# DiamondLightSource/fast-feedback-service

Hardware: AMD Instinct MI355X
Metric: detector frames/s (Eiger-16M 4362x4148 uint16) (higher is better)
Workload: dtype u16; 1 GPU; eiger16m: 4148x4362 uint16, 7x7 dispersion window, 32 frames/step/GPU resident in HBM, spots+centroids returned to host; streams=4, parallelism=single GPU, spot_gather=none (single GPU)

## Files before the change

fast-feedback-service_amd/csrc/ffs_context.hip:

```cpp
#include <sys/mman.h>

#include "ffs_internal.hpp"
#include "kernels_mask.hpp"

static_assert(sizeof(ReflOut) == sizeof(ffs_reflection), "record layout");
static_assert(offsetof(ReflOut, sum_intensity) == offsetof(ffs_reflection, sum_intensity), "record layout");

thread_local std::string g_create_error;

static void ctx_destroy_internal(ffs_ctx* c);
namespace {
struct Registry {
    std::mutex mu;
    std::unordered_set<const void*> live[3];
    std::atomic<bool> exiting{false};
    bool exit_hook_installed = false;
};
Registry& registry() {
    static Registry* r = new Registry();
    return *r;
}
static void on_process_exit() {
    Registry& r = registry();
    std::vector<ffs_ctx*> ctxs;
// ... 131 lines not shown
    L.bpitch = (uint32_t)L.pitch_px;
    L.frame_stride = (uint64_t)L.pitch * height;
    L.plane_frame_stride = (uint64_t)L.mpitch * height;
    L.bytes_frame_stride = (uint64_t)L.bpitch * height;
    if (L.frame_stride >= (1ull << 32)) {
        g_create_error = "frame larger than 4 GiB";
        delete c;
        return FFS_ERR_INVALID;
    }
    const uint64_t npx = (uint64_t)width * height;
    c->cap = max_strong ? max_strong : (uint32_t)std::min<uint64_t>(npx, 1u << 18);
    c->cap = (uint32_t)std::min<uint64_t>(c->cap, npx);
    c->max_comp = std::min<uint32_t>(c->cap, 1u << 14);
    c->n_tiles = ((int)height + kTileRows - 1) / kTileRows;
    ffs_default_params(&c->params);
    if (hipSetDevice(device) != hipSuccess) {
        g_create_error = "hipSetDevice failed";
        delete c;
        return FFS_ERR_DEVICE;
    }
    hipError_t e = hipMalloc(&c->d_maskbits, L.plane_frame_stride + 256);
    if (e == hipSuccess) e = hipMalloc(&c->d_ginfo, (size_t)(L.H + kInfoExtraRows) * ((size_t)L.pitch_px * pixel_bytes / 4) + 256);
    if (e == hipSuccess) e = hipMalloc(&c->d_mmap, (size_t)L.H * L.pitch_px + 256);
    if (e != hipSuccess) {
        g_create_error = std::string("hipMalloc(mask): ") + hipGetErrorString(e);
        ctx_destroy_internal(c);
        return FFS_ERR_NOMEM;
    }
    c->chain_ok = chain_prepare_device();
    {
        int lo = 0, hi = 0;
        hipError_t es = hipDeviceGetStreamPriorityRange(&lo, &hi);
        if (es == hipSuccess) es = hipStreamCreateWithPriority(&c->dense_st, hipStreamNonBlocking, (lo + hi) / 2);
        if (es == hipSuccess) es = hipStreamCreateWithFlags(&c->up_st, hipStreamNonBlocking);
        for (auto& sp : c->sparse_st)
            if (es == hipSuccess) es = hipStreamCreateWithPriority(&sp, hipStreamNonBlocking, hi);
        if (es == hipSuccess)
            for (auto& e : c->chain_ev)
                if (es == hipSuccess) es = hipEventCreate(&e);
        if (es != hipSuccess) {
            g_create_error = std::string("creating the context's HIP streams: ") + hipGetErrorString(es);
            ctx_destroy_internal(c);
            return FFS_ERR_DEVICE;
        }
    }
    int rc = ffs_ctx_set_mask(c, nullptr);
// ... 80 lines not shown
    for (ffs_stream* s : streams)
        if (handle_take(kHandleStream, s)) stream_destroy_internal(s);
    for (ffs_stack3d* st : stacks)
        if (handle_take(kHandleStack, st)) {
            g_live_stacks.fetch_sub(1);
            stack3d_free(st);
        }
    ctx_destroy_internal(c);
}

static void ctx_destroy_internal(ffs_ctx* c) {
    (void)hipSetDevice(c->device);
    ahead_stop(c, true);
    for (auto* st : c->stack_pool) stack3d_free(st);
    c->stack_pool.clear();
    if (AssemblyPool* pool = c->assembly.exchange(nullptr)) {
        pool->owner.lock();
        pool->owner.unlock();
        delete pool;
    }
    if (c->d_maskbits) (void)hipFree(c->d_maskbits);
    if (c->d_ginfo) (void)hipFree(c->d_ginfo);
    if (c->d_mmap) (void)hipFree(c->d_mmap);
    if (c->dense_st) (void)hipStreamDestroy(c->dense_st);
    if (c->dense_st2) (void)hipStreamDestroy(c->dense_st2);
    if (c->d_handoff) (void)hipFree(c->d_handoff);
    if (c->up_st) (void)hipStreamDestroy(c->up_st);
    for (auto st : c->sparse_st) if (st) (void)hipStreamDestroy(st);
    for (auto e : c->chain_ev) if (e) (void)hipEventDestroy(e);
    for (auto& pb : c->pinned_pool) pinned_free(pb);
    delete c;
}

static int rebuild_mask_tables(ffs_ctx* c) {
    const Layout& L = c->L;
    const uint32_t gpitch = (uint32_t)L.pitch_px * (uint32_t)c->pixel_bytes / 4;
    HIP_TRY(c, hipMemset(c->d_ginfo, 0, (size_t)(L.H + kInfoExtraRows) * gpitch));
    const int groups = L.pitch_px / (c->pixel_bytes == 2 ? 8 : 4);
    (void)hipGetLastError();
    if (c->pixel_bytes == 2)
        hipLaunchKernelGGL(k_build_maps, dim3((groups + 255) / 256, L.H), dim3(256), 0, 0, c->d_maskbits, L.mpitch, L.W, L.H,
                           L.pitch_px, c->d_mmap, c->d_ginfo, gpitch);
    else
        hipLaunchKernelGGL(k_build_maps4, dim3((groups + 255) / 256, L.H), dim3(256), 0, 0, c->d_maskbits, L.mpitch, L.W, L.H,
                           L.pitch_px, c->d_mmap, c->d_ginfo, gpitch);
    HIP_TRY(c, hipGetLastError());
    HIP_TRY(c, hipDeviceSynchronize());
    return FFS_OK;
}

static int ffs_ctx_set_mask_impl(ffs_ctx* c, const uint8_t* host_mask) {
    if (!c) return FFS_ERR_INVALID;
    const Layout& L = c->L;
    std::vector<uint8_t> bits(L.plane_frame_stride, 0);
    const int full = L.W / 8;
    for (int y = 0; y < L.H; ++y) {
        uint8_t* row = bits.data() + (size_t)y * L.mpitch;
        if (host_mask) {
            const uint8_t* m = host_mask + (size_t)y * L.W;
            for (int g = 0; g < full; ++g) {
                uint64_t v;
                std::memcpy(&v, m + 8 * g, 8);
                const uint64_t nz = (((v & 0x7F7F7F7F7F7F7F7Full) + 0x7F7F7F7F7F7F7F7Full) | v) & 0x8080808080808080ull;
                row[g] = (uint8_t)(((nz >> 7) * 0x0102040810204080ull) >> 56);
            }
            for (int x = full * 8; x < L.W; ++x)
                if (m[x]) row[x >> 3] |= (uint8_t)(1u << (x & 7));
        } else {
// ... 60 lines not shown

extern "C" int ffs_ctx_device_layout(const ffs_ctx* c, size_t* pitch, size_t* fstride) {
    if (!c) return FFS_ERR_INVALID;
    if (pitch) *pitch = c->L.pitch;
    if (fstride) *fstride = c->L.frame_stride;
    return FFS_OK;
}

extern "C" int ffs_ctx_set_tuning(ffs_ctx* c, const char* key, long long value) {
    if (!c || !key) return FFS_ERR_INVALID;
    Tuning& t = c->tune;
    const std::string k = key;
    auto in = [&](long long lo, long long hi) { return value >= lo && value <= hi; };
    bool ok = true;
    if (k == "threshold_path") { if ((ok = in(0, 2))) t.threshold_path = (int)value; }
    else if (k == "window_kernel") { if ((ok = in(0, 1))) t.window_kernel = (int)value; }
    else if (k == "ext_first_pass") { if ((ok = value == 0 || value == 2)) t.ext_first_pass = (int)value; }
    else if (k == "sparse_stage") { if ((ok = in(1, 3))) t.sparse_stage = (int)value; }
    else if (k == "device_lists") { if ((ok = in(0, 2))) t.device_lists = (int)value; }
    else if (k == "strong_log") { if ((ok = in(0, 1))) t.strong_log = (int)value; }
    else if (k == "chain_runs") { if ((ok = in(0, 2))) t.chain_runs = (int)value; }
    else if (k == "dense_overlap") { if ((ok = in(0, 1))) t.dense_overlap = (int)value; }
    else if (k == "stream_prio") { if ((ok = in(0, 3))) t.stream_prio = (int)value; }
    else if (k == "wait_ahead") { if ((ok = in(0, 1))) t.wait_ahead = (int)value; }
    else if (k == "assembly_threads") { if ((ok = in(1, 31))) t.assembly_threads = (int)value; }
    else if (k == "sparse_bands") { if ((ok = in(0, 2))) t.sparse_bands = (int)value; }
    else if (k == "sparse_priority") {
        if ((ok = in(0, 2) && c->n_streams_made == 0)) {
            int lo = 0, hi = 0;
            HIP_TRY(c, hipSetDevice(c->device));
            HIP_TRY(c, hipDeviceGetStreamPriorityRange(&lo, &hi));
            const int prio = value == 0 ? hi : value == 1 ? lo : (lo + hi) / 2;
            for (auto& sp : c->sparse_st) {
                if (sp) (void)hipStreamDestroy(sp);
                sp = nullptr;
                HIP_TRY(c, hipStreamCreateWithPriority(&sp, hipStreamNonBlocking, prio));
            }
            t.sparse_priority = (int)value;
        }
    }
    else if (k == "sched") { if ((ok = (value == 0 || value == 3) && c->n_streams_made == 0)) t.sched = (int)value; }
    else if (k == "chain_first") { if ((ok = in(0, 64))) t.chain_first = (int)value; }
    else if (k == "bright_cap") { if ((ok = in(0, kBrightCap))) t.bright_cap = (int)value; }
    else if (k == "frames_per_group") { if ((ok = in(1, 1 << 30))) t.frames_per_group = (int)value; }
    else if (k == "target_waves") { if ((ok = in(1, 1 << 24))) t.target_waves = value; }
    else if (k == "stream_bands") { if ((ok = in(0, 4096))) t.stream_bands = (int)value; }
// ... 284 lines not shown
```

fast-feedback-service_amd/csrc/ffs_device.h:

```cpp
#pragma once
#include <hip/hip_runtime.h>
#include <stdint.h>

#ifdef FFS_EXPERIMENTS
#define FFS_DBG(args, bit) (((args).dbg & (bit)) != 0)
#define FFS_STOP_AFTER(A, phase) if ((A).stop_after == (phase)) return
#define FFS_PHASE_TS(A, idx) do { if ((A).phase_ts && threadIdx.x == 0) (A).phase_ts[(size_t)blockIdx.x * 8 + (idx)] = wall_clock64(); } while (0)
#else
#define FFS_PHASE_TS(A, idx) do {} while (0)
#define FFS_DBG(args, bit) false
#define FFS_STOP_AFTER(A, phase) do {} while (0)
#endif

namespace ffsamd {

struct Layout {
    int W, H;
    int pitch_px;
    uint32_t pitch;
    uint32_t mpitch;
    uint32_t bpitch;
    uint64_t frame_stride;
    uint64_t plane_frame_stride;
    uint64_t bytes_frame_stride;
};

constexpr int kSOwned = 62;
__host__ __device__ inline int band_first_row(int band, int band_rows, int band_rows2, int band_split) {
    return band < band_split ? band * band_rows : band_split * band_rows + (band - band_split) * band_rows2;
}
constexpr int kWinOwned = 62;
constexpr int kInfoExtraRows = 3;

constexpr int kWlogCap = 256;
constexpr int kTileRows = 8;
constexpr int kExactListCap = 2048;

struct ThresholdArgs {
    const void* image;
    uint64_t frame_stride;
    uint32_t pitch;
    const uint8_t* maskbits;
    uint8_t* bits;
    uint8_t* strong_bytes;
    uint32_t* tile_counts;
    int W, H, pitch_px;
    uint32_t mpitch, bpitch;
    uint64_t plane_frame_stride, bytes_frame_stride;
    int n_strips, band_rows, n_bands, n_tiles;
    int band_rows2, band_split;
    float kS;
    float kB;
    int min_count;
    double nsig_b, nsig_s, threshold;
    double nsig_b2, nsig_s2;
    long long max_valid;
    int int_pred;
    uint32_t ib2, is2;
    uint32_t thr_floor;
    int bright_to_plane;
    uint8_t* dplane;
    uint8_t* eplane;
    int eplane_clean;
    int ext_strips, ext_band_rows, ext_bands;
    int ext_flavour;
    int ext_variant;
    const uint8_t* ginfo;
    const uint8_t* mmap;
    uint32_t gpitch;
    int gpf;
    int n_frames;
    int group_frames;
    int s_strips, s_band_rows, s_bands;
    uint32_t* bright_n;
    uint2* bright_list;
    uint32_t bright_cap;
    uint32_t* overflow;
    uint32_t* occ;
    uint32_t occ_frame_words;
    uint32_t occ_spr;
    int dense_mask;
    uint2* wlog;
    uint32_t* wlog_n;
    uint4* wpix;
    uint32_t* handoff;
    uint32_t handoff_seq;
    int dbg_prio;
    int dbg;
    int kx, ky;
    int w_strips, w_band_rows, w_bands;
    float w_kS, w_kB;
};
// ... 148 lines not shown
```

fast-feedback-service_amd/csrc/ffs_internal.hpp:

```cpp
#pragma once
#include <algorithm>
#include <atomic>
#include <chrono>
#include <condition_variable>
#include <functional>
#include <cmath>
#include <cstdio>
#include <cstdlib>
#include <cstring>
#include <deque>
#include <map>
#include <mutex>
#include <new>
#include <string>
#include <thread>
#include <unordered_set>
#include <vector>

#include <hip/hip_runtime.h>
#include <hip/hip_ext.h>

#include "ffs_hip.h"
#include "ffs_device.h"

// ... 19 lines not shown
    int sched = 3;
    int chain_first = 2;
    int bright_cap = 1 << 20;
    int frames_per_group = 1 << 30;
    long long target_waves = 16384;
    int stream_bands = 0;
    int dense_mask = 0;
    int occupancy_bitmap = 1;
    int direct_records = 1;
    int decode_in_dense_stream = 1;
    int ccl_grid = 32;
    int ext_erode = 2;
    int ext_e_sparse = 0;
    int ext_fused = 0;
    int ext_rest_aside = 0;
    int band_taper = 0;
    int rows_ahead = 3;
    int device_lists = 2;
    int strong_log = 1;
    int chain_runs = 1;
    int sparse_bands = 1;
    int dense_overlap = 0;
    int stream_prio = 1;
    int assembly_threads = 7;
    int wait_ahead = 1;
    int sparse_priority = 0;
    int window_kernel = 0;
#ifdef FFS_EXPERIMENTS
    struct Exp {
        int k1_debug = 0, chain_skip = 0, chain_stop = 0, dummy_us = 0, dummy_wg = 32, dummy_threads = 1024, dummy_lds = 0;
    } exp;
#endif
};

struct ffs_stack3d;

struct AssemblyPool {
    std::vector<std::thread> threads;
    std::mutex mu;
    std::condition_variable cv;
    std::mutex owner;
    const std::function<void(uint32_t)>* job = nullptr;
    uint32_t n_items = 0;
    std::atomic<uint32_t> next{0}, done{0};
    std::atomic<int> active{0};
    uint64_t generation = 0;
// ... 14 lines not shown
void pinned_free(PinnedBuf& b);

struct AheadThread {
    std::thread th;
    std::mutex mu;
    std::condition_variable cv_work, cv_done;
    std::deque<ffs_stream*> q;
    bool stop = false;
};

struct ffs_ctx {
    int device = 0;
    Tuning tune;
    Layout L{};
    int pixel_bytes = 2;
    uint32_t max_batch = 1;
    uint32_t cap = 0;
    uint32_t max_comp = 0;
    int n_tiles = 0;
    ffs_params params{};
    uint8_t* d_maskbits = nullptr;
    uint8_t* d_ginfo = nullptr;
    uint8_t* d_mmap = nullptr;
    hipStream_t dense_st = nullptr;
    hipStream_t dense_st2 = nullptr;
    uint32_t* d_handoff = nullptr;
    std::mutex dense_mu;
    uint32_t handoff_seq = 0;
    int handoff_last = -1;
    hipStream_t up_st = nullptr;
    hipStream_t sparse_st[2] = {nullptr, nullptr};
    int n_streams_made = 0;
    std::mutex stream_mu;
    std::vector<ffs_stream*> live_streams;
    std::vector<ffs_stack3d*> live_stacks;
    std::vector<ffs_stack3d*> stack_pool;
    std::vector<struct PinnedBuf> pinned_pool;
    std::atomic<int> inflight{0};
    static constexpr int kChainEvents = 16;
    hipEvent_t chain_ev[kChainEvents] = {};
    std::atomic<uint32_t> chain_ev_next{0};
    std::atomic<int> chain_ev_newest{-1};
    bool chain_ok = false;
    std::atomic<AssemblyPool*> assembly{nullptr};
    std::atomic<AheadThread*> ahead{nullptr};
    ThreadError err;
// ... 209 lines not shown
```

fast-feedback-service_amd/csrc/ffs_submit.hip:

```cpp
#include "ffs_internal.hpp"
#include "kernels_threshold.hpp"
#include "kernels_extended.hpp"
#include "kernels_stream.hpp"
#include "kernels_ccl.hpp"
#include "kernels_chain.hpp"
#include "kernels_band.hpp"
#include "kernels_decode.hpp"
#include "kernels_window.hpp"

bool chain_prepare_device() {
    const hipError_t e1 = hipFuncSetAttribute(reinterpret_cast<const void*>(&k_frame_chain<uint16_t>), hipFuncAttributeMaxDynamicSharedMemorySize, kChainDynBytes);
    const hipError_t e2 = hipFuncSetAttribute(reinterpret_cast<const void*>(&k_frame_chain<uint32_t>), hipFuncAttributeMaxDynamicSharedMemorySize, kChainDynBytes);
    const hipError_t e3 = hipFuncSetAttribute(reinterpret_cast<const void*>(&k_frame_chain<uint16_t, true>), hipFuncAttributeMaxDynamicSharedMemorySize, kChainDynBytes);
    const hipError_t e4 = hipFuncSetAttribute(reinterpret_cast<const void*>(&k_frame_chain<uint16_t, false, true>), hipFuncAttributeMaxDynamicSharedMemorySize, kChainDynBytes);
    const hipError_t e5 = hipFuncSetAttribute(reinterpret_cast<const void*>(&k_frame_chain<uint32_t, false, true>), hipFuncAttributeMaxDynamicSharedMemorySize, kChainDynBytes);
    (void)hipGetLastError();
    return e1 == hipSuccess && e2 == hipSuccess && e3 == hipSuccess && e4 == hipSuccess && e5 == hipSuccess;
}

ThresholdArgs make_threshold_args(ffs_stream* s, const void* img, size_t pitch, size_t fstride, uint32_t n_frames, const Rerun& how) {
    const ffs_ctx* c = s->ctx;
    const Layout& L = c->L;
    const ffs_params& p = s->batch_params;
    ThresholdArgs a{};
// ... 26 lines not shown
        a.int_pred = (b2 == std::floor(b2) && s2 == std::floor(s2) && b2 <= 1024.0 && s2 <= 1024.0 && p.threshold < 2147483648.0
                      && std::sqrt(b2) == p.nsig_b && std::sqrt(s2) == p.nsig_s) ? 1 : 0;
        a.ib2 = a.int_pred ? (uint32_t)b2 : 0u;
        a.is2 = a.int_pred ? (uint32_t)s2 : 0u;
        a.thr_floor = a.int_pred ? (uint32_t)std::floor(p.threshold) : 0u;
    }
    a.bright_to_plane = how.threshold_path >= 0 ? how.threshold_path : c->tune.threshold_path;
    a.overflow = s->d_overflow;
    a.bright_n = s->d_tile_counts + tile_counts_bytes(s) / 4 - 1;
    a.bright_list = s->d_bright;
    a.bright_cap = std::min<uint32_t>(kBrightCap, (uint32_t)c->tune.bright_cap);
    a.occ = s->d_occ;
    a.occ_frame_words = occ_frame_words(L);
    a.occ_spr = L.mpitch / 16;
    a.dense_mask = (p.want_strong_mask || c->tune.dense_mask || a.bright_to_plane) ? 1 : 0;
#ifdef FFS_EXPERIMENTS
    a.dbg = c->tune.exp.k1_debug;
    if (a.dbg & 16) a.dense_mask = 1;
    if (a.dbg & 8) a.dense_mask = 0;
#endif
    a.dbg_prio = c->tune.stream_prio;
    a.ginfo = c->d_ginfo;
    a.mmap = c->d_mmap;
    a.gpitch = (uint32_t)L.pitch_px * (uint32_t)c->pixel_bytes / 4;
    a.gpf = c->pixel_bytes == 2 ? (L.W + 7) / 8 : (L.W + 3) / 4;
    a.n_frames = (int)n_frames;
    {
        const uint64_t per_frame = std::max<uint64_t>(fstride, L.bytes_frame_stride);
        a.group_frames = (int)std::max<uint64_t>(1, std::min<uint64_t>(n_frames, ((1ull << 31) - 1) / per_frame));
        a.group_frames = std::min(a.group_frames, c->tune.frames_per_group);
        const int n_groups = ((int)n_frames + a.group_frames - 1) / a.group_frames;
        const long long lanes = (long long)a.group_frames * (a.gpf + 1);
        const long long lines = (long long)a.group_frames * (L.bpitch / 128);
        const int lines_per_wave = c->pixel_bytes == 2 ? 4 : 2;
        a.n_strips = (int)std::max<long long>((lanes + kSOwned - 1) / kSOwned, (lines + lines_per_wave - 1) / lines_per_wave);
        const long long per_band = std::max<long long>(1, (long long)a.n_strips * n_groups);
        long long nb = std::max<long long>(1, std::min<long long>(c->tune.target_waves / per_band, L.H / 72));
        if (nb >= 8) nb = nb / 8 * 8;
        if (c->tune.stream_bands > 0) nb = std::max<long long>(1, std::min<long long>(c->tune.stream_bands, L.H / 8));
        a.band_rows = (int)std::min<long long>(1024, (L.H + nb - 1) / nb);
        a.n_bands = (L.H + a.band_rows - 1) / a.band_rows;
        a.band_rows2 = a.band_rows;
        a.band_split = a.n_bands;
        const int taper = c->tune.band_taper;
        if (taper > 0 && taper < 100 && nb >= 32 && nb % 8 == 0 && a.n_bands == (int)nb) {
            const int K = (int)nb / 8;
// ... 1009 lines not shown
```

fast-feedback-service_amd/csrc/kernels_mask.hpp:

```cpp
#pragma once
#include "ffs_device.h"

namespace ffsamd {

__global__ __launch_bounds__(256) void k_build_maps(const uint8_t* maskbits, uint32_t mpitch, int W, int H, int pitch_px,
                                                    uint8_t* mmap, uint8_t* ginfo, uint32_t gpitch_bytes) {
    const int g = blockIdx.x * 256 + threadIdx.x;
    const int y = blockIdx.y;
    if (g * 8 >= pitch_px) return;
    uint32_t cnt[8] = {0, 0, 0, 0, 0, 0, 0, 0};
    for (int dy = -3; dy <= 3; ++dy) {
        const int yy = y + dy;
        if (yy < 0 || yy >= H) continue;
        const uint8_t* row = maskbits + (uint64_t)yy * mpitch;
        uint32_t b = (uint32_t)row[g] << 8;
        if (g > 0) b |= row[g - 1];
        if ((uint32_t)(g + 1) < mpitch) b |= (uint32_t)row[g + 1] << 16;
        for (int j = 0; j < 8; ++j) cnt[j] += __popc((b >> (j + 5)) & 0x7Fu);
    }
    const uint32_t own = maskbits[(uint64_t)y * mpitch + g];
    uint32_t mn = 255, mx = 0;
    for (int j = 0; j < 8; ++j) {
        mmap[(uint64_t)y * pitch_px + g * 8 + j] = (uint8_t)cnt[j];
        if ((own >> j) & 1u) { mn = min(mn, cnt[j]); mx = max(mx, cnt[j]); }
// ... 14 lines not shown
    const int byte0 = (g * 4) >> 3, sh = (g * 4) & 7;
    for (int dy = -3; dy <= 3; ++dy) {
        const int yy = y + dy;
        if (yy < 0 || yy >= H) continue;
        const uint8_t* row = maskbits + (uint64_t)yy * mpitch;
        uint32_t b = (uint32_t)row[byte0] << 8;
        if (byte0 > 0) b |= row[byte0 - 1];
        if ((uint32_t)(byte0 + 1) < mpitch) b |= (uint32_t)row[byte0 + 1] << 16;
        for (int j = 0; j < 4; ++j) cnt[j] += __popc((b >> (5 + sh + j)) & 0x7Fu);
    }
    const uint32_t own = (maskbits[(uint64_t)y * mpitch + byte0] >> sh) & 0xFu;
    uint32_t mn = 255, mx = 0;
    for (int j = 0; j < 4; ++j) {
        mmap[(uint64_t)y * pitch_px + g * 4 + j] = (uint8_t)cnt[j];
        if ((own >> j) & 1u) { mn = min(mn, cnt[j]); mx = max(mx, cnt[j]); }
    }
    if (mx == 0) mn = 0;
    ginfo[(uint64_t)y * gpitch_bytes + g * 4] = (uint8_t)own;
    ginfo[(uint64_t)(y + kInfoExtraRows) * gpitch_bytes + g * 4 + 1] = (uint8_t)mn;
    ginfo[(uint64_t)(y + kInfoExtraRows) * gpitch_bytes + g * 4 + 2] = (uint8_t)mx;
    ginfo[(uint64_t)(y + kInfoExtraRows) * gpitch_bytes + g * 4 + 3] = (uint8_t)own;
}


__global__ void k_resolution_mask(uint8_t* maskbits, uint32_t mpitch, int W, int H, float wavelength,
                                  float distance, float cx, float cy, float psx, float psy,
                                  float dmin, float dmax) {
    const int bx = blockIdx.x * blockDim.x + threadIdx.x;
    const int y = blockIdx.y;
    if (bx * 8 >= W || y >= H) return;
    uint8_t* p = maskbits + (uint64_t)y * mpitch + bx;
    uint32_t b = *p;
    for (int j = 0; j < 8; ++j) {
        const int x = bx * 8 + j;
        if (x >= W || !((b >> j) & 1u)) continue;
        const float dx = (((float)x + 0.5f) - cx) * psx;
        const float dy = (((float)y + 0.5f) - cy) * psy;
        const float r = sqrtf(dx * dx + dy * dy);
        const float theta = 0.5f * atanf(r / distance);
        const float res = wavelength / (2.0f * sinf(theta));
        if ((dmin > 0 && res < dmin) || (dmax > 0 && res > dmax)) b &= ~(1u << j);
    }
    *p = (uint8_t)b;
}

}
// ... 1 lines not shown
```

fast-feedback-service_amd/csrc/kernels_stream.hpp:

```cpp
#pragma once
#include "kernels_threshold.hpp"

#ifndef FFS_IMG_LOAD_AUX
#define FFS_IMG_LOAD_AUX 0
#endif

namespace ffsamd {

constexpr int kSQWords = 32;

__device__ __forceinline__ bool exact_predicate(const ThresholdArgs& a, uint32_t m, unsigned long long sx,
                                                unsigned long long sy, uint32_t pc) {
    const double src = (double)pc;
    if (!((int)m >= a.min_count && src > a.threshold)) return false;
    if (a.max_valid >= 0 && (long long)pc > a.max_valid) return false;
    const double md = (double)m, xd = (double)sx, yd = (double)sy;
    const double t0 = md * yd;
    const double t1 = xd * xd;
    const double t2 = xd * (md - 1.0);
    const double av = (t0 - t1) - t2;
    const double bv = md * src - xd;
    const double cv = (xd * a.nsig_b) * __builtin_sqrt(2.0 * (md - 1.0));
    const double dv = a.nsig_s * __builtin_sqrt(xd * md);
    return av > cv && bv > dv;
// ... 39 lines not shown

__device__ __forceinline__ bool dispersion_only(const ThresholdArgs& a, uint32_t m, unsigned long long sx, unsigned long long sy) {
    const double md = (double)m, xd = (double)sx, yd = (double)sy;
    const double t0 = md * yd;
    const double t1 = xd * xd;
    const double t2 = xd * (md - 1.0);
    const double av = (t0 - t1) - t2;
    const double cv = (xd * a.nsig_b) * __builtin_sqrt(2.0 * (md - 1.0));
    return av > cv;
}
__device__ __forceinline__ bool dispersion_only_nosqrt(const ThresholdArgs& a, uint32_t m, unsigned long long sx, unsigned long long sy,
                                                       bool& certain) {
    certain = true;
    const double md = (double)m, xd = (double)sx, yd = (double)sy;
    const double av = (md * yd - xd * xd) - xd * (md - 1.0);
    if (!(av > 0.0)) return false;
    const double a2 = av * av, c2 = (a.nsig_b2 * (xd * xd)) * (2.0 * (md - 1.0));
    constexpr double kEps = 9.094947017729282e-13;
    const bool yes = a2 > c2 + c2 * kEps, no = a2 < c2 - c2 * kEps;
    certain = yes || no;
    return yes;
}

__device__ __forceinline__ uint32_t dpp_shr_add(uint32_t from_neighbour, uint32_t addend) {
    return (uint32_t)__builtin_amdgcn_update_dpp(0, (int)from_neighbour, 0x138, 0xf, 0xf, true) + addend;
}
__device__ __forceinline__ uint32_t dpp_shl_add(uint32_t from_neighbour, uint32_t addend) {
    return (uint32_t)__builtin_amdgcn_update_dpp(0, (int)from_neighbour, 0x130, 0xf, 0xf, true) + addend;
}


template <int KAHEAD, bool EXT = false, bool DENSE = false>
__global__ __launch_bounds__(64, 4) void k_stream_u16(const ThresholdArgs a) {
    __shared__ uint32_t s_q[kSQWords][kQCap];
    __shared__ uint16_t s_list[kQCap * 8];

    const int lane = threadIdx.x;
    if (a.dbg_prio & 1) __builtin_amdgcn_s_setprio(3);
    int strip, band;
    const bool real = stream_unit(a, blockIdx.x, strip, band);
    if constexpr (!EXT)
        if (a.handoff && blockIdx.x == gridDim.x - 1 && blockIdx.y == gridDim.y - 1 && lane == 0)
            __hip_atomic_store(a.handoff, a.handoff_seq, __ATOMIC_RELEASE, __HIP_MEMORY_SCOPE_SYSTEM);
    if (!real) return;
    [[maybe_unused]] const uint32_t slot = log_slot(a, blockIdx.y, (uint32_t)band, (uint32_t)strip);
    const int f0 = blockIdx.y * a.group_frames;
// ... 8 lines not shown
    const bool active = G >= 0 && fl < nf && g < a.gpf;
    const bool owned = active && lane >= 1 && lane <= kSOwned;
    const uint32_t my_fg = ((uint32_t)fl << 16) | (uint32_t)g;

    const rsrc_t r_img = make_rsrc((const uint8_t*)a.image + (uint64_t)f0 * a.frame_stride,
                                   (uint32_t)((uint64_t)(nf - 1) * a.frame_stride + (uint64_t)a.H * a.pitch));
    const rsrc_t r_info = make_rsrc(a.ginfo, (uint32_t)(a.H + kInfoExtraRows) * a.gpitch);
    const rsrc_t r_sb = make_rsrc(a.strong_bytes + (uint64_t)f0 * a.bytes_frame_stride,
                                  (uint32_t)((uint64_t)nf * a.bytes_frame_stride));
    const rsrc_t r_cb = make_rsrc((EXT ? a.dplane : a.bits) + (uint64_t)f0 * a.plane_frame_stride, (uint32_t)((uint64_t)nf * a.plane_frame_stride));
    constexpr uint32_t kOob = 0x80000000u;
    const uint32_t off_px = active ? (uint32_t)((uint64_t)fl * a.frame_stride) + (uint32_t)g * 16u : kOob;
    const uint32_t off_info = active ? (uint32_t)g * 4u : kOob;
    uint32_t off_byte_st;
    {
        const uint32_t lpf = a.bpitch >> 7;
        const uint32_t u = (uint32_t)strip * 4u + ((uint32_t)lane >> 4);
        const uint32_t fz = u / lpf, cz = u - fz * lpf;
        off_byte_st = fz < (uint32_t)nf ? (uint32_t)((uint64_t)fz * a.bytes_frame_stride) + cz * 128u + ((uint32_t)lane & 15u) * 8u : kOob;
    }

    const int total = (yb1 - yb0) + (FFS_DBG(a, 1024) ? 0 : 6);
    const float kS = a.kS;

    constexpr int NS = 7 + KAHEAD;
    uint32_t ring[NS][4];
    uint32_t rinfo[NS];
    uint32_t col[8], colq[8];
    uint32_t M[4] = {0, 0, 0, 0};
    uint32_t mprev = 0;
    typedef float f32x2 __attribute__((ext_vector_type(2)));
    [[maybe_unused]] f32x2 ext_c1 = {0.0f, 0.0f}, ext_c2 = {0.0f, 0.0f};
#pragma unroll
    for (int s = 0; s < NS; ++s) {
        rinfo[s] = 0;
#pragma unroll
        for (int q = 0; q < 4; ++q) ring[s][q] = 0;
    }
#pragma unroll
    for (int j = 0; j < 8; ++j) { col[j] = 0; colq[j] = 0; }
    const unsigned long long owned_mask = __builtin_amdgcn_ballot_w64(owned);

    auto fetch = [&](int slot, int i) {
        const int yin = yb0 - 3 + i;
        const uint32_t prow = (uint32_t)min(max(yin, 0), a.H - 1);
        const uint32_t irow = (uint32_t)min(max(yin, 0), a.H + kInfoExtraRows - 1);
        const u32x4 v = __builtin_amdgcn_raw_buffer_load_b128(r_img, off_px, prow * a.pitch, FFS_IMG_LOAD_AUX);
        ring[slot][0] = v[0]; ring[slot][1] = v[1]; ring[slot][2] = v[2]; ring[slot][3] = v[3];
        rinfo[slot] = __builtin_amdgcn_raw_buffer_load_b32(r_info, off_info | (yin < 0 ? kOob : 0u), (FFS_DBG(a, 64) ? 8u : irow) * a.gpitch, 0);
    };

    auto mask_row = [&](int slot, int slot_before) {
        if (__ballot(rinfo[slot] != rinfo[slot_before]) != 0ull) {
            const uint32_t mb = rinfo[slot] & 0xFFu;
            if (__ballot(mb != mprev) != 0ull) {
#pragma unroll
                for (int q = 0; q < 4; ++q)
                    M[q] = ((uint32_t)__builtin_amdgcn_sbfe((int)mb, 2 * q, 1) & 0xFFFFu)
                         | ((uint32_t)__builtin_amdgcn_sbfe((int)mb, 2 * q + 1, 1) & 0xFFFF0000u);
                mprev = mb;
            }
            if constexpr (EXT) {
                const uint32_t mmin = (rinfo[slot] >> 8) & 0xFFu, mmax = (rinfo[slot] >> 16) & 0xFFu;
                const float mm1 = (float)mmin - 1.0f;
                const float c1 = (float)mmax * 1.0000019073486328125f;
                const float c2 = (mm1 + a.kB * __builtin_amdgcn_sqrtf(2.0f * mm1)) * 0.99999952316284179688f;
                ext_c1 = f32x2{c1, c1};
                ext_c2 = f32x2{c2, c2};
            }
        }
#pragma unroll
        for (int q = 0; q < 4; ++q) {
            ring[slot][q] &= M[q];
            asm("" : "+v"(ring[slot][q]));
        }
    };

    auto push = [&](int s, int so) {
#pragma unroll
        for (int q = 0; q < 4; ++q) {
            const uint32_t wn = ring[s][q], wo = ring[so][q];
            {
                const int32_t t = (int32_t)((wn & 0xFFFFu) - (wo & 0xFFFFu));
                const int32_t u = (int32_t)((wn & 0xFFFFu) + (wo & 0xFFFFu));
                col[2 * q] += (uint32_t)t;
                colq[2 * q] += (uint32_t)__mul24(t, u);
            }
            {
                const int32_t t = (int32_t)((wn >> 16) - (wo >> 16));
                const int32_t u = (int32_t)((wn >> 16) + (wo >> 16));
                col[2 * q + 1] += (uint32_t)t;
                colq[2 * q + 1] += (uint32_t)__mul24(t, u);
            }
// ... 144 lines not shown
                if ((uint32_t)lane - nbuf < cnt) {
                    lbuf[0] = e0; lbuf[1] = e1;
                    lbuf[2] = p0; lbuf[3] = p1; lbuf[4] = p2; lbuf[5] = p3;
                }
                nbuf += cnt;
            }
            qn = 0;
            return;
        }
        if (have) {
            const uint32_t cb = s_q[14][lane];
            if (cb) {
                if (!FFS_DBG(a, 256)) __builtin_amdgcn_raw_buffer_store_b8((uint8_t)cb, r_cb, (uint32_t)((uint64_t)fe * a.plane_frame_stride) + ge, row * a.mpitch, 0);
                if constexpr (!EXT) if (!FFS_DBG(a, 128)) {
                    atomicAdd(a.tile_counts + (uint64_t)(f0 + (int)fe) * a.n_tiles + (row / (uint32_t)kTileRows), (uint32_t)__popc(cb));
                    const uint32_t ob = row * a.occ_spr + (ge >> 4);
                    atomicOr(a.occ + (uint64_t)(f0 + (int)fe) * a.occ_frame_words + (ob >> 5), 1u << (ob & 31u));
                }
            }
        }
        qn = 0;
    };

#pragma unroll
    for (int s = 0; s < KAHEAD; ++s) fetch(s, s);

#pragma unroll
    for (int s = 0; s < 6; ++s) {
        mask_row(s, (s + NS - 1) % NS);
        push(s, (s + KAHEAD) % NS);
        fetch((s + KAHEAD) % NS, s + KAHEAD);
    }

    for (int base = 6;; base += NS) {
#pragma unroll
        for (int t = 0; t < NS; ++t) {
            const int s = (6 + t) % NS;
            const int so = (s + KAHEAD) % NS;
            const int sc = (s + NS - 3) % NS;
            const int i = base + t;
            if (i >= total) goto rows_done;
            {
                const uint32_t info = rinfo[s];
                mask_row(s, (s + NS - 1) % NS);
                push(s, so);
                fetch(so, i + KAHEAD);

                const uint32_t s01 = col[0] + col[1], s23 = col[2] + col[3], s45 = col[4] + col[5], s67 = col[6] + col[7];
                const uint32_t ua = s01 + s23, va = s45 + s67;
                const uint32_t T0 = dpp_shr_add(s67, ua);
                const uint32_t T1 = ua + s45;
                const uint32_t T2 = va + s23;
                const uint32_t T3 = dpp_shl_add(s01, va);
                uint32_t Wn[8];
                Wn[0] = dpp_shr_add(col[5], T0);
                Wn[1] = T0 + col[4];
                Wn[2] = dpp_shr_add(col[7], T1);
                Wn[3] = T1 + col[6];
                Wn[4] = T2 + col[1];
                Wn[5] = dpp_shl_add(col[0], T2);
                Wn[6] = T3 + col[3];
                Wn[7] = dpp_shl_add(col[2], T3);

                const int yout = __builtin_amdgcn_readfirstlane(yb0 + (i - 6));
                const uint32_t so_bytes = (uint32_t)yout * a.bpitch;

                const uint32_t xmin = min(min(min(min(Wn[0], Wn[1]), Wn[2]), min(min(Wn[3], Wn[4]), Wn[5])), min(Wn[6], Wn[7]));
                const uint32_t mmin = (info >> 8) & 0xFFu, mmax = (info >> 16) & 0xFFu;
                bool pass;
                [[maybe_unused]] uint32_t ys[8];
                if constexpr (EXT) {
                    const uint32_t q01 = colq[0] + colq[1], q23 = colq[2] + colq[3], q45 = colq[4] + colq[5], q67 = colq[6] + colq[7];
                    const uint32_t qa = q01 + q23, qb = q45 + q67;
                    const uint32_t U0 = dpp_shr_add(q67, qa), U1 = qa + q45, U2 = qb + q23, U3 = dpp_shl_add(q01, qb);
                    const uint32_t y0 = dpp_shr_add(colq[5], U0), y1 = U0 + colq[4], y2 = dpp_shr_add(colq[7], U1), y3 = U1 + colq[6];
                    const uint32_t y4 = U2 + colq[1], y5 = dpp_shl_add(colq[0], U2), y6 = U3 + colq[3], y7 = dpp_shl_add(colq[2], U3);
                    ys[0] = y0; ys[1] = y1; ys[2] = y2; ys[3] = y3; ys[4] = y4; ys[5] = y5; ys[6] = y6; ys[7] = y7;
                    float dmax = -1.0f;
#pragma unroll
                    for (int jp = 0; jp < 4; ++jp) {
                        const f32x2 xf = {(float)Wn[2 * jp], (float)Wn[2 * jp + 1]};
                        const f32x2 yf = {(float)ys[2 * jp], (float)ys[2 * jp + 1]};
                        const f32x2 u = xf * (xf + ext_c2);
                        const f32x2 d = __builtin_elementwise_fma(ext_c1, yf, -u);
                        dmax = __builtin_fmaxf(dmax, __builtin_fmaxf(d.x, d.y));
                    }
                    const uint32_t xmax = max(max(max(max(Wn[0], Wn[1]), Wn[2]), max(max(Wn[3], Wn[4]), Wn[5])), max(Wn[6], Wn[7]));
                    pass = mmax != 0u && (dmax >= 0.0f || xmax >= 65536u);
                } else {
                    uint32_t pmax;
                    {
                        typedef uint16_t u16x2 __attribute__((ext_vector_type(2)));
                        const u16x2 a01 = __builtin_bit_cast(u16x2, ring[sc][0]), a23 = __builtin_bit_cast(u16x2, ring[sc][1]);
                        const u16x2 a45 = __builtin_bit_cast(u16x2, ring[sc][2]), a67 = __builtin_bit_cast(u16x2, ring[sc][3]);
                        const u16x2 mx = __builtin_elementwise_max(__builtin_elementwise_max(a01, a23), __builtin_elementwise_max(a45, a67));
                        const uint32_t mw = __builtin_bit_cast(uint32_t, mx);
                        pmax = max(mw & 0xFFFFu, mw >> 16);
                    }
                    const int32_t B = (int32_t)__umul24(mmax, pmax) - (int32_t)xmin;
                    const float bf = (float)B, tf = (float)__umul24(xmin, mmin);
                    float lhs = bf * __builtin_fabsf(bf);
                    asm("" : "+v"(lhs));
                    pass = lhs > kS * tf;
                }
                if constexpr (DENSE) __builtin_amdgcn_raw_buffer_store_b64(u32x2{0u, 0u}, r_sb, off_byte_st, so_bytes, 2 );
                const unsigned long long fm = FFS_DBG(a, 1) ? 0ull : (__builtin_amdgcn_ballot_w64(pass) & owned_mask);
                const bool flag = pass && owned;
                if (fm) {
                    const int nfl = __popcll(fm);
                    if (qn + nfl > kQCap) drain();
                    if constexpr (EXT) {
                        if (flag && !FFS_DBG(a, 32)) {
                            const uint32_t rank = __builtin_amdgcn_mbcnt_hi((uint32_t)(fm >> 32), __builtin_amdgcn_mbcnt_lo((uint32_t)fm, 0u));
                            const int e = qn + (int)rank;
#pragma unroll
                            for (int w = 0; w < 8; ++w) {
                                s_q[w][e] = Wn[w];
                                s_q[16 + w][e] = ys[w];
                            }
#pragma unroll
                            for (int w = 0; w < 4; ++w) s_q[8 + w][e] = ring[sc][w];
                            s_q[15][e] = info;
                            s_q[30][e] = ((uint32_t)yout << 6) | (uint32_t)lane; s_q[31][e] = my_fg;
                        }
                    } else {
                    const uint32_t QL5 = from_left(colq[5]), QL6 = from_left(colq[6]), QL7 = from_left(colq[7]);
                    const uint32_t QR0 = from_right(colq[0]), QR1 = from_right(colq[1]), QR2 = from_right(colq[2]);
                    if (flag && !FFS_DBG(a, 32)) {
// ... 69 lines not shown
    const int fl = G >= 0 ? G / gsep : 0;
    const int g = G - fl * gsep;
    const bool active = G >= 0 && fl < nf && g < a.gpf;
    const bool owned = active && lane >= 1 && lane <= kSOwned;

    const rsrc_t r_img = make_rsrc((const uint8_t*)a.image + (uint64_t)f0 * a.frame_stride,
                                   (uint32_t)((uint64_t)(nf - 1) * a.frame_stride + (uint64_t)a.H * a.pitch));
    const rsrc_t r_info = make_rsrc(a.ginfo, (uint32_t)(a.H + kInfoExtraRows) * a.gpitch);
    const rsrc_t r_sb = make_rsrc(a.strong_bytes + (uint64_t)f0 * a.bytes_frame_stride,
                                  (uint32_t)((uint64_t)nf * a.bytes_frame_stride));
    constexpr uint32_t kOob = 0x80000000u;
    const uint32_t off_px = active ? (uint32_t)((uint64_t)fl * a.frame_stride) + (uint32_t)g * 16u : kOob;
    const uint32_t off_info = active ? (uint32_t)g * 4u : kOob;
    uint32_t off_byte_st;
    {
        const uint32_t lpf = a.bpitch >> 7;
        const uint32_t u = (uint32_t)strip * 2u + ((uint32_t)lane >> 4);
        const uint32_t fz = u / lpf, cz = u - fz * lpf;
        off_byte_st = (lane < 32 && fz < (uint32_t)nf) ? (uint32_t)((uint64_t)fz * a.bytes_frame_stride) + cz * 128u + ((uint32_t)lane & 15u) * 8u : kOob;
    }

    const int total = (yb1 - yb0) + 6;
    const float kS = a.kS;

    constexpr int NS = 7 + KAHEAD;
    uint32_t ring[NS][4];
    uint32_t rinfo[NS];
    uint32_t col[4];
    long long colq[4];
    uint32_t M[4] = {0, 0, 0, 0};
    uint32_t mprev = 0;
    uint32_t bighist = 0;
#pragma unroll
    for (int s = 0; s < NS; ++s) {
        rinfo[s] = 0;
#pragma unroll
        for (int q = 0; q < 4; ++q) ring[s][q] = 0;
    }
#pragma unroll
    for (int j = 0; j < 4; ++j) { col[j] = 0; colq[j] = 0; }
    const unsigned long long owned_mask = __builtin_amdgcn_ballot_w64(owned);

    auto fetch = [&](int slot, int i) {
        const int yin = yb0 - 3 + i;
        const uint32_t prow = (uint32_t)min(max(yin, 0), a.H - 1);
        const uint32_t irow = (uint32_t)min(max(yin, 0), a.H + kInfoExtraRows - 1);
        const u32x4 v = __builtin_amdgcn_raw_buffer_load_b128(r_img, off_px, prow * a.pitch, FFS_IMG_LOAD_AUX);
        ring[slot][0] = v[0]; ring[slot][1] = v[1]; ring[slot][2] = v[2]; ring[slot][3] = v[3];
        rinfo[slot] = __builtin_amdgcn_raw_buffer_load_b32(r_info, off_info | (yin < 0 ? kOob : 0u), irow * a.gpitch, 0);
    };

    auto mask_row = [&](int slot, int slot_before) {
        if (__ballot(rinfo[slot] != rinfo[slot_before]) != 0ull) {
            const uint32_t mb = rinfo[slot] & 0xFu;
            if (__ballot(mb != mprev) != 0ull) {
#pragma unroll
                for (int q = 0; q < 4; ++q) M[q] = (uint32_t)__builtin_amdgcn_sbfe((int)mb, q, 1);
                mprev = mb;
            }
        }
#pragma unroll
        for (int q = 0; q < 4; ++q) ring[slot][q] &= M[q];
    };

    auto push = [&](int s, int so) {
        const uint32_t big = ((ring[s][0] | ring[s][1]) | (ring[s][2] | ring[s][3])) >> 24 ? 1u : 0u;
        bighist = (bighist & ~((1u << s) | (1u << so))) | (big << s);
#pragma unroll
        for (int q = 0; q < 4; ++q) {
            const int32_t t = (int32_t)(ring[s][q] - ring[so][q]), u = (int32_t)(ring[s][q] + ring[so][q]);
            col[q] += (uint32_t)t;
            colq[q] += (long long)t * (long long)u;
        }
    };

    int qn = 0;
    uint32_t nlog = 0;
    uint32_t nbuf = 0;
    uint32_t lbuf[6] = {0, 0, 0, 0, 0, 0};
    auto flush_log = [&]() {
        const uint32_t at = nlog + (uint32_t)lane;
        if ((uint32_t)lane < nbuf && at < (uint32_t)kWlogCap) {
            a.wlog[(uint64_t)slot * kWlogCap + at] = make_uint2(lbuf[0], lbuf[1]);
            a.wpix[(uint64_t)slot * kWlogCap + at] = make_uint4(lbuf[2], lbuf[3], lbuf[4], lbuf[5]);
        }
        nlog += nbuf;
        nbuf = 0;
    };
    auto drain = [&]() {
        const bool have = lane < qn && !FFS_DBG(a, 2) && !FFS_DBG(a, 32);
        uint32_t todo = 0, row = 0, fe = 0, ge = 0, info = 0;
        bool big = false;
        if (have) {
            const uint32_t tag = s_q[11][lane], ln = tag & 63u;
            big = (tag >> 31) != 0u;
            row = (tag & 0x7FFFFFFFu) >> 6;
            const int Ge = strip * kSOwned + (int)ln - 1;
// ... 83 lines not shown
                if ((uint32_t)lane - nbuf < cnt) {
                    lbuf[0] = e0; lbuf[1] = e1;
                    lbuf[2] = p0; lbuf[3] = p1; lbuf[4] = p2; lbuf[5] = p3;
                }
                nbuf += cnt;
            }
            qn = 0;
            return;
        }
        if (have) {
            const uint32_t cb = s_q[10][lane];
            if (cb) {
                const uint32_t x0 = ge * 4u;
                uint32_t* plane = reinterpret_cast<uint32_t*>(a.bits + (uint64_t)(f0 + (int)fe) * a.plane_frame_stride + (uint64_t)row * a.mpitch);
                atomicOr(plane + (x0 >> 5), cb << (x0 & 31u));
                atomicAdd(a.tile_counts + (uint64_t)(f0 + (int)fe) * a.n_tiles + (row / (uint32_t)kTileRows), (uint32_t)__popc(cb));
                const uint32_t ob = row * a.occ_spr + (x0 >> 7);
                atomicOr(a.occ + (uint64_t)(f0 + (int)fe) * a.occ_frame_words + (ob >> 5), 1u << (ob & 31u));
            }
        }
        qn = 0;
    };

#pragma unroll
    for (int s = 0; s < KAHEAD; ++s) fetch(s, s);
#pragma unroll
    for (int s = 0; s < 6; ++s) {
        mask_row(s, (s + NS - 1) % NS);
        push(s, (s + KAHEAD) % NS);
        fetch((s + KAHEAD) % NS, s + KAHEAD);
    }

    for (int base = 6;; base += NS) {
#pragma unroll
        for (int t = 0; t < NS; ++t) {
            const int s = (6 + t) % NS;
            const int so = (s + KAHEAD) % NS;
            const int sc = (s + NS - 3) % NS;
            const int i = base + t;
            if (i >= total) goto rows_done;
            {
                const uint32_t info = rinfo[s];
                mask_row(s, (s + NS - 1) % NS);
                push(s, so);
                fetch(so, i + KAHEAD);

                const uint32_t s01 = col[0] + col[1], s23 = col[2] + col[3];
                const uint32_t S = s01 + s23;
                const uint32_t TL = dpp_shr_add(s23, S);
                const uint32_t TR = dpp_shl_add(s01, S);
                uint32_t Wn[4];
                Wn[0] = dpp_shr_add(col[1], TL);
                Wn[1] = dpp_shl_add(col[0], TL);
                Wn[2] = dpp_shr_add(col[3], TR);
                Wn[3] = dpp_shl_add(col[2], TR);

                const int yout = __builtin_amdgcn_readfirstlane(yb0 + (i - 6));
                if constexpr (DENSE) __builtin_amdgcn_raw_buffer_store_b64(u32x2{0u, 0u}, r_sb, off_byte_st, (uint32_t)yout * a.bpitch, 2);

                const uint32_t xmin = min(min(min(Wn[0], Wn[1]), Wn[2]), Wn[3]);
                const uint32_t pmax = max(max(max(ring[sc][0], ring[sc][1]), ring[sc][2]), ring[sc][3]);
                const uint32_t mmin = (info >> 8) & 0xFFu, mmax = (info >> 16) & 0xFFu;
                const int32_t B = (int32_t)(mmax * pmax) - (int32_t)xmin;
                const float bf = (float)B, tf = (float)xmin * (float)mmin;
                const bool pass = bf * __builtin_fabsf(bf) > kS * tf;
                const uint32_t bl = bighist != 0u ? 1u : 0u;
                bool near_big = false;
                if (__ballot(bl != 0u) != 0ull) near_big = (bl | from_left(bl) | from_right(bl)) != 0u && mmax != 0u;
                const bool want = pass || near_big;
                const unsigned long long fm = FFS_DBG(a, 1) ? 0ull : (__builtin_amdgcn_ballot_w64(want) & owned_mask);
                const bool flag = want && owned;
                if (fm) {
                    const int nfl = __popcll(fm);
                    if (qn + nfl > kQCap) drain();
                    uint32_t ql[4], qh[4];
#pragma unroll
                    for (int w = 0; w < 4; ++w) { ql[w] = (uint32_t)colq[w]; qh[w] = (uint32_t)((unsigned long long)colq[w] >> 32); }
                    const uint32_t QL1 = from_left(ql[1]), QL2 = from_left(ql[2]), QL3 = from_left(ql[3]);
                    const uint32_t QR0 = from_right(ql[0]), QR1 = from_right(ql[1]), QR2 = from_right(ql[2]);
                    const uint32_t HL1 = from_left(qh[1]), HL2 = from_left(qh[2]), HL3 = from_left(qh[3]);
                    const uint32_t HR0 = from_right(qh[0]), HR1 = from_right(qh[1]), HR2 = from_right(qh[2]);
// ... 46 lines not shown
```

Measured before the change: 110,400 frames/s.

## Skip image loads and window math for fully masked detector rows

Builds a per-row dead table from the mask, stored as sliding 32-bit windows, and uses it in the streaming dispersion kernels. Dead rows get out-of-bounds buffer loads so no memory is read. Their masking and column push are skipped when both the entering and leaving rows are dead, and the centre-row threshold work is skipped when the output row is dead. Eiger has horizontal module gaps, so this aims to cut bandwidth and ALU on those rows, at the cost of an extra scalar load per iteration and more branching in the unrolled loop.

```diff
diff --git a/fast-feedback-service_amd/csrc/ffs_context.hip b/fast-feedback-service_amd/csrc/ffs_context.hip
--- a/fast-feedback-service_amd/csrc/ffs_context.hip
+++ b/fast-feedback-service_amd/csrc/ffs_context.hip
@@ -177,6 +177,7 @@
     hipError_t e = hipMalloc(&c->d_maskbits, L.plane_frame_stride + 256);
     if (e == hipSuccess) e = hipMalloc(&c->d_ginfo, (size_t)(L.H + kInfoExtraRows) * ((size_t)L.pitch_px * pixel_bytes / 4) + 256);
     if (e == hipSuccess) e = hipMalloc(&c->d_mmap, (size_t)L.H * L.pitch_px + 256);
+    if (e == hipSuccess) e = hipMalloc(&c->d_rowdead, 2 * (size_t)dead_words(L.H) * sizeof(uint32_t));
     if (e != hipSuccess) {
         g_create_error = std::string("hipMalloc(mask): ") + hipGetErrorString(e);
         ctx_destroy_internal(c);
@@ -303,6 +304,7 @@
     if (c->d_maskbits) (void)hipFree(c->d_maskbits);
     if (c->d_ginfo) (void)hipFree(c->d_ginfo);
     if (c->d_mmap) (void)hipFree(c->d_mmap);
+    if (c->d_rowdead) (void)hipFree(c->d_rowdead);
     if (c->dense_st) (void)hipStreamDestroy(c->dense_st);
     if (c->dense_st2) (void)hipStreamDestroy(c->dense_st2);
     if (c->d_handoff) (void)hipFree(c->d_handoff);
@@ -325,6 +327,11 @@
     else
         hipLaunchKernelGGL(k_build_maps4, dim3((groups + 255) / 256, L.H), dim3(256), 0, 0, c->d_maskbits, L.mpitch, L.W, L.H,
                            L.pitch_px, c->d_mmap, c->d_ginfo, gpitch);
+    HIP_TRY(c, hipGetLastError());
+    const uint32_t nw = dead_words(L.H);
+    HIP_TRY(c, hipMemset(c->d_rowdead, 0xFF, (size_t)nw * sizeof(uint32_t)));
+    HIP_TRY(c, hipMemset(c->d_rowdead + nw, 0, (size_t)nw * sizeof(uint32_t)));
+    hipLaunchKernelGGL(k_build_row_dead, dim3(L.H), dim3(64), 0, 0, c->d_maskbits, L.mpitch, L.H, c->d_rowdead, nw);
     HIP_TRY(c, hipGetLastError());
     HIP_TRY(c, hipDeviceSynchronize());
     return FFS_OK;
@@ -431,6 +438,7 @@
     else if (k == "chain_runs") { if ((ok = in(0, 2))) t.chain_runs = (int)value; }
     else if (k == "dense_overlap") { if ((ok = in(0, 1))) t.dense_overlap = (int)value; }
     else if (k == "stream_prio") { if ((ok = in(0, 3))) t.stream_prio = (int)value; }
+    else if (k == "skip_dead_rows") { if ((ok = in(0, 1))) t.skip_dead_rows = (int)value; }
     else if (k == "wait_ahead") { if ((ok = in(0, 1))) t.wait_ahead = (int)value; }
     else if (k == "assembly_threads") { if ((ok = in(1, 31))) t.assembly_threads = (int)value; }
     else if (k == "sparse_bands") { if ((ok = in(0, 2))) t.sparse_bands = (int)value; }
diff --git a/fast-feedback-service_amd/csrc/ffs_device.h b/fast-feedback-service_amd/csrc/ffs_device.h
--- a/fast-feedback-service_amd/csrc/ffs_device.h
+++ b/fast-feedback-service_amd/csrc/ffs_device.h
@@ -31,6 +31,9 @@
 }
 constexpr int kWinOwned = 62;
 constexpr int kInfoExtraRows = 3;
+constexpr int kDeadPad = 16;
+constexpr int kDeadExtraWords = 64;
+__host__ __device__ inline uint32_t dead_words(int H) { return (uint32_t)(H + kDeadPad + kDeadExtraWords); }
 
 constexpr int kWlogCap = 256;
 constexpr int kTileRows = 8;
@@ -68,6 +71,7 @@
     const uint8_t* ginfo;
     const uint8_t* mmap;
     uint32_t gpitch;
+    const uint32_t* row_dead;
     int gpf;
     int n_frames;
     int group_frames;
diff --git a/fast-feedback-service_amd/csrc/ffs_internal.hpp b/fast-feedback-service_amd/csrc/ffs_internal.hpp
--- a/fast-feedback-service_amd/csrc/ffs_internal.hpp
+++ b/fast-feedback-service_amd/csrc/ffs_internal.hpp
@@ -65,6 +65,7 @@
     int sparse_bands = 1;
     int dense_overlap = 0;
     int stream_prio = 1;
+    int skip_dead_rows = 1;
     int assembly_threads = 7;
     int wait_ahead = 1;
     int sparse_priority = 0;
@@ -125,6 +126,7 @@
     uint8_t* d_maskbits = nullptr;
     uint8_t* d_ginfo = nullptr;
     uint8_t* d_mmap = nullptr;
+    uint32_t* d_rowdead = nullptr;
     hipStream_t dense_st = nullptr;
     hipStream_t dense_st2 = nullptr;
     uint32_t* d_handoff = nullptr;
diff --git a/fast-feedback-service_amd/csrc/ffs_submit.hip b/fast-feedback-service_amd/csrc/ffs_submit.hip
--- a/fast-feedback-service_amd/csrc/ffs_submit.hip
+++ b/fast-feedback-service_amd/csrc/ffs_submit.hip
@@ -72,6 +72,7 @@
     a.dbg_prio = c->tune.stream_prio;
     a.ginfo = c->d_ginfo;
     a.mmap = c->d_mmap;
+    a.row_dead = c->d_rowdead + (c->tune.skip_dead_rows ? 0u : dead_words(L.H));
     a.gpitch = (uint32_t)L.pitch_px * (uint32_t)c->pixel_bytes / 4;
     a.gpf = c->pixel_bytes == 2 ? (L.W + 7) / 8 : (L.W + 3) / 4;
     a.n_frames = (int)n_frames;
diff --git a/fast-feedback-service_amd/csrc/kernels_mask.hpp b/fast-feedback-service_amd/csrc/kernels_mask.hpp
--- a/fast-feedback-service_amd/csrc/kernels_mask.hpp
+++ b/fast-feedback-service_amd/csrc/kernels_mask.hpp
@@ -60,6 +60,16 @@
     ginfo[(uint64_t)(y + kInfoExtraRows) * gpitch_bytes + g * 4 + 3] = (uint8_t)own;
 }
 
+__global__ __launch_bounds__(64) void k_build_row_dead(const uint8_t* maskbits, uint32_t mpitch, int H, uint32_t* row_dead, uint32_t n_words) {
+    const int y = blockIdx.x;
+    const uint32_t* row = reinterpret_cast<const uint32_t*>(maskbits + (uint64_t)y * mpitch);
+    uint32_t any = 0;
+    for (uint32_t w = threadIdx.x; w < mpitch / 4; w += 64) any |= row[w];
+    if (__ballot(any != 0u) == 0ull) return;
+    const int b = (int)threadIdx.x;
+    const int k = y + kDeadPad - b;
+    if (b < 32 && k >= 0 && (uint32_t)k < n_words) atomicAnd(row_dead + k, ~(1u << b));
+}
 
 __global__ void k_resolution_mask(uint8_t* maskbits, uint32_t mpitch, int W, int H, float wavelength,
                                   float distance, float cx, float cy, float psx, float psy,
diff --git a/fast-feedback-service_amd/csrc/kernels_stream.hpp b/fast-feedback-service_amd/csrc/kernels_stream.hpp
--- a/fast-feedback-service_amd/csrc/kernels_stream.hpp
+++ b/fast-feedback-service_amd/csrc/kernels_stream.hpp
@@ -85,6 +85,8 @@
     return yes;
 }
 
+typedef const __attribute__((address_space(4))) uint32_t* dead_ptr_t;
+
 __device__ __forceinline__ uint32_t dpp_shr_add(uint32_t from_neighbour, uint32_t addend) {
     return (uint32_t)__builtin_amdgcn_update_dpp(0, (int)from_neighbour, 0x138, 0xf, 0xf, true) + addend;
 }
@@ -139,6 +141,7 @@
 
     const int total = (yb1 - yb0) + (FFS_DBG(a, 1024) ? 0 : 6);
     const float kS = a.kS;
+    const dead_ptr_t dead_tab = (dead_ptr_t)a.row_dead + (yb0 - 3 + kDeadPad);
 
     constexpr int NS = 7 + KAHEAD;
     uint32_t ring[NS][4];
@@ -158,16 +161,16 @@
     for (int j = 0; j < 8; ++j) { col[j] = 0; colq[j] = 0; }
     const unsigned long long owned_mask = __builtin_amdgcn_ballot_w64(owned);
 
-    auto fetch = [&](int slot, int i) {
+    auto fetch = [&](int slot, int i, bool dead) {
         const int yin = yb0 - 3 + i;
         const uint32_t prow = (uint32_t)min(max(yin, 0), a.H - 1);
         const uint32_t irow = (uint32_t)min(max(yin, 0), a.H + kInfoExtraRows - 1);
-        const u32x4 v = __builtin_amdgcn_raw_buffer_load_b128(r_img, off_px, prow * a.pitch, FFS_IMG_LOAD_AUX);
+        const u32x4 v = __builtin_amdgcn_raw_buffer_load_b128(r_img, off_px | (dead ? kOob : 0u), prow * a.pitch, FFS_IMG_LOAD_AUX);
         ring[slot][0] = v[0]; ring[slot][1] = v[1]; ring[slot][2] = v[2]; ring[slot][3] = v[3];
         rinfo[slot] = __builtin_amdgcn_raw_buffer_load_b32(r_info, off_info | (yin < 0 ? kOob : 0u), (FFS_DBG(a, 64) ? 8u : irow) * a.gpitch, 0);
     };
 
-    auto mask_row = [&](int slot, int slot_before) {
+    auto track_mask = [&](int slot, int slot_before) {
         if (__ballot(rinfo[slot] != rinfo[slot_before]) != 0ull) {
             const uint32_t mb = rinfo[slot] & 0xFFu;
             if (__ballot(mb != mprev) != 0ull) {
@@ -186,6 +189,8 @@
                 ext_c2 = f32x2{c2, c2};
             }
         }
+    };
+    auto mask_row = [&](int slot) {
 #pragma unroll
         for (int q = 0; q < 4; ++q) {
             ring[slot][q] &= M[q];
@@ -376,17 +381,22 @@
         qn = 0;
     };
 
-#pragma unroll
-    for (int s = 0; s < KAHEAD; ++s) fetch(s, s);
+    const uint32_t dw = dead_tab[0];
+#pragma unroll
+    for (int s = 0; s < KAHEAD; ++s) fetch(s, s, (dw >> s) & 1u);
 
 #pragma unroll
     for (int s = 0; s < 6; ++s) {
-        mask_row(s, (s + NS - 1) % NS);
-        push(s, (s + KAHEAD) % NS);
-        fetch((s + KAHEAD) % NS, s + KAHEAD);
+        track_mask(s, (s + NS - 1) % NS);
+        if (!((dw >> s) & 1u)) {
+            mask_row(s);
+            push(s, (s + KAHEAD) % NS);
+        }
+        fetch((s + KAHEAD) % NS, s + KAHEAD, (dw >> (s + KAHEAD)) & 1u);
     }
 
     for (int base = 6;; base += NS) {
+        const uint32_t db = dead_tab[base - 7];
 #pragma unroll
         for (int t = 0; t < NS; ++t) {
             const int s = (6 + t) % NS;
@@ -395,10 +405,21 @@
             const int i = base + t;
             if (i >= total) goto rows_done;
             {
+                const uint32_t kVert = (1u << (t + 7)) | (1u << t);
+                const bool skip_vert = (db & kVert) == kVert;
+                const bool skip_centre = (db >> (t + 4)) & 1u;
                 const uint32_t info = rinfo[s];
-                mask_row(s, (s + NS - 1) % NS);
-                push(s, so);
-                fetch(so, i + KAHEAD);
+                track_mask(s, (s + NS - 1) % NS);
+                if (!skip_vert) {
+                    mask_row(s);
+                    push(s, so);
+                }
+                fetch(so, i + KAHEAD, (db >> (t + 7 + KAHEAD)) & 1u);
+
+                const int yout = __builtin_amdgcn_readfirstlane(yb0 + (i - 6));
+                [[maybe_unused]] const uint32_t so_bytes = (uint32_t)yout * a.bpitch;
+                if constexpr (DENSE) __builtin_amdgcn_raw_buffer_store_b64(u32x2{0u, 0u}, r_sb, off_byte_st, so_bytes, 2 );
+                if (skip_centre) continue;
 
                 const uint32_t s01 = col[0] + col[1], s23 = col[2] + col[3], s45 = col[4] + col[5], s67 = col[6] + col[7];
                 const uint32_t ua = s01 + s23, va = s45 + s67;
@@ -415,9 +436,6 @@
                 Wn[5] = dpp_shl_add(col[0], T2);
                 Wn[6] = T3 + col[3];
                 Wn[7] = dpp_shl_add(col[2], T3);
-
-                const int yout = __builtin_amdgcn_readfirstlane(yb0 + (i - 6));
-                const uint32_t so_bytes = (uint32_t)yout * a.bpitch;
 
                 const uint32_t xmin = min(min(min(min(Wn[0], Wn[1]), Wn[2]), min(min(Wn[3], Wn[4]), Wn[5])), min(Wn[6], Wn[7]));
                 const uint32_t mmin = (info >> 8) & 0xFFu, mmax = (info >> 16) & 0xFFu;
@@ -457,7 +475,6 @@
                     asm("" : "+v"(lhs));
                     pass = lhs > kS * tf;
                 }
-                if constexpr (DENSE) __builtin_amdgcn_raw_buffer_store_b64(u32x2{0u, 0u}, r_sb, off_byte_st, so_bytes, 2 );
                 const unsigned long long fm = FFS_DBG(a, 1) ? 0ull : (__builtin_amdgcn_ballot_w64(pass) & owned_mask);
                 const bool flag = pass && owned;
                 if (fm) {
@@ -573,6 +590,7 @@
 
     const int total = (yb1 - yb0) + 6;
     const float kS = a.kS;
+    const dead_ptr_t dead_tab = (dead_ptr_t)a.row_dead + (yb0 - 3 + kDeadPad);
 
     constexpr int NS = 7 + KAHEAD;
     uint32_t ring[NS][4];
@@ -592,16 +610,16 @@
     for (int j = 0; j < 4; ++j) { col[j] = 0; colq[j] = 0; }
     const unsigned long long owned_mask = __builtin_amdgcn_ballot_w64(owned);
 
-    auto fetch = [&](int slot, int i) {
+    auto fetch = [&](int slot, int i, bool dead) {
         const int yin = yb0 - 3 + i;
         const uint32_t prow = (uint32_t)min(max(yin, 0), a.H - 1);
         const uint32_t irow = (uint32_t)min(max(yin, 0), a.H + kInfoExtraRows - 1);
-        const u32x4 v = __builtin_amdgcn_raw_buffer_load_b128(r_img, off_px, prow * a.pitch, FFS_IMG_LOAD_AUX);
+        const u32x4 v = __builtin_amdgcn_raw_buffer_load_b128(r_img, off_px | (dead ? kOob : 0u), prow * a.pitch, FFS_IMG_LOAD_AUX);
         ring[slot][0] = v[0]; ring[slot][1] = v[1]; ring[slot][2] = v[2]; ring[slot][3] = v[3];
         rinfo[slot] = __builtin_amdgcn_raw_buffer_load_b32(r_info, off_info | (yin < 0 ? kOob : 0u), irow * a.gpitch, 0);
     };
 
-    auto mask_row = [&](int slot, int slot_before) {
+    auto track_mask = [&](int slot, int slot_before) {
         if (__ballot(rinfo[slot] != rinfo[slot_before]) != 0ull) {
             const uint32_t mb = rinfo[slot] & 0xFu;
             if (__ballot(mb != mprev) != 0ull) {
@@ -610,6 +628,8 @@
                 mprev = mb;
             }
         }
+    };
+    auto mask_row = [&](int slot) {
 #pragma unroll
         for (int q = 0; q < 4; ++q) ring[slot][q] &= M[q];
     };
@@ -624,6 +644,7 @@
             colq[q] += (long long)t * (long long)u;
         }
     };
+    auto push_dead = [&](int s, int so) { bighist &= ~((1u << s) | (1u << so)); };
 
     int qn = 0;
     uint32_t nlog = 0;
@@ -753,16 +774,23 @@
         qn = 0;
     };
 
-#pragma unroll
-    for (int s = 0; s < KAHEAD; ++s) fetch(s, s);
+    const uint32_t dw = dead_tab[0];
+#pragma unroll
+    for (int s = 0; s < KAHEAD; ++s) fetch(s, s, (dw >> s) & 1u);
 #pragma unroll
     for (int s = 0; s < 6; ++s) {
-        mask_row(s, (s + NS - 1) % NS);
-        push(s, (s + KAHEAD) % NS);
-        fetch((s + KAHEAD) % NS, s + KAHEAD);
+        track_mask(s, (s + NS - 1) % NS);
+        if (!((dw >> s) & 1u)) {
+            mask_row(s);
+            push(s, (s + KAHEAD) % NS);
+        } else {
+            push_dead(s, (s + KAHEAD) % NS);
+        }
+        fetch((s + KAHEAD) % NS, s + KAHEAD, (dw >> (s + KAHEAD)) & 1u);
     }
 
     for (int base = 6;; base += NS) {
+        const uint32_t db = dead_tab[base - 7];
 #pragma unroll
         for (int t = 0; t < NS; ++t) {
             const int s = (6 + t) % NS;
@@ -771,10 +799,20 @@
             const int i = base + t;
             if (i >= total) goto rows_done;
             {
+                const uint32_t kVert = (1u << (t + 7)) | (1u << t);
                 const uint32_t info = rinfo[s];
-                mask_row(s, (s + NS - 1) % NS);
-                push(s, so);
-                fetch(so, i + KAHEAD);
+                track_mask(s, (s + NS - 1) % NS);
+                if ((db & kVert) != kVert) {
+                    mask_row(s);
+                    push(s, so);
+                } else {
+                    push_dead(s, so);
+                }
+                fetch(so, i + KAHEAD, (db >> (t + 7 + KAHEAD)) & 1u);
+
+                const int yout = __builtin_amdgcn_readfirstlane(yb0 + (i - 6));
+                if constexpr (DENSE) __builtin_amdgcn_raw_buffer_store_b64(u32x2{0u, 0u}, r_sb, off_byte_st, (uint32_t)yout * a.bpitch, 2);
+                if ((db >> (t + 4)) & 1u) continue;
 
                 const uint32_t s01 = col[0] + col[1], s23 = col[2] + col[3];
                 const uint32_t S = s01 + s23;
@@ -785,9 +823,6 @@
                 Wn[1] = dpp_shl_add(col[0], TL);
                 Wn[2] = dpp_shr_add(col[3], TR);
                 Wn[3] = dpp_shl_add(col[2], TR);
-
-                const int yout = __builtin_amdgcn_readfirstlane(yb0 + (i - 6));
-                if constexpr (DENSE) __builtin_amdgcn_raw_buffer_store_b64(u32x2{0u, 0u}, r_sb, off_byte_st, (uint32_t)yout * a.bpitch, 2);
 
                 const uint32_t xmin = min(min(min(Wn[0], Wn[1]), Wn[2]), Wn[3]);
                 const uint32_t pmax = max(max(max(ring[sc][0], ring[sc][1]), ring[sc][2]), ring[sc][3]);
```

Measured after the change: 100,000 frames/s. 9.4% lower.
